# ryhorv/tf-flowavenet

Hardware: AMD Instinct MI355X
Metric: audio samples/sec: forward NLL + inverse synth, n_block=8 bf16 (higher is better)
Workload: dtype bf16; 1 GPU; configs[1]: full model n_block=8 n_flow=6 n_layer=2, forward NLL + inverse synthesis, 16128-sample (63-frame) clips @22.05 kHz; clips_per_gpu=8, samples_per_clip=16128, weights=synthetic seed 1234, ActNorm DDI on the first (global) batch, parallelism=batch shard x1, no data-path collective (2-scalar NLL all-reduce), streams=7 per direction

## Files before the change

### tf-flowavenet_amd/csrc/flow_kernels.hip

```cpp
#include "common.h"
#include "gemm_ring.h"
#include "fwn_internal.h"

struct RowCtxT {
    int row;
    int t;
};

struct FrontProb {
    static constexpr bool A_DMA = false;
    const float* xa;
    const float* an;
    const bf16* W;
    const float* bias;
    bf16* hout;
    int M, Ti, Ch, chlog, kpad, apply_an;
    unsigned char* h8out = nullptr;
    typedef RowCtxT RowCtx;
    struct ChunkCtx { int k0; int lo; };
    __device__ int nchunks() const { return 2 * (kpad / FWN_BK); }
    __device__ RowCtx row_ctx(int row) const { return RowCtx{row, row % Ti}; }
    __device__ ChunkCtx chunk_ctx(int q) const {
        const int nk = kpad / FWN_BK;
        const int lo = q >= nk;
// ... 540 lines not shown
                if (h8out) {
                    const srd_t s8 = make_srd(h8out, (uint32_t)((size_t)M * FWN_HID));
#pragma unroll
                    for (int r = 0; r < 16; r += 2) {
                        const unsigned int pk = pack_e4m3x2((float)(bf16)((hv[r] + acc[mi][ni][r] + b) * 0.70710678118654752f),
                                                            (float)(bf16)((hv[r + 1] + acc[mi][ni][r + 1] + b) * 0.70710678118654752f));
                        buf_store_u8(s8, voff >> 1, (uint32_t)((mi * 32 + acc_row_c(r)) * FWN_HID), pk);
                        buf_store_u8(s8, voff >> 1, (uint32_t)((mi * 32 + acc_row_c(r + 1)) * FWN_HID), pk >> 8);
                    }
                }
            }
        }
    }
};

struct CondProb {
    static constexpr bool NT_B = true;
    static constexpr bool A_DMA = true;
    static constexpr bool ALLOW_256 = false;
    const bf16* ca;
    const bf16* Wc;
    float* P;
    int M, cin, kcpad;
    int k_begin = 0, k_end = 0;
    struct RowCtx { int row; };
    struct ChunkCtx { int k0; };
    template <int BK> __device__ int nchunks() const { return ((k_end ? k_end : kcpad) - k_begin) / BK; }
    __device__ RowCtx row_ctx(int row) const { return RowCtx{row}; }
    template <int BK> __device__ ChunkCtx chunk_ctx(int q) const { return ChunkCtx{k_begin + q * BK}; }
    __device__ srd_t a_srd(const ChunkCtx&) const { return make_srd(ca, (uint32_t)((size_t)M * cin * 2)); }
    __device__ uint32_t a_voff(const ChunkCtx& cc, const RowCtx& rc, int c8) const {
        const bool ok = rc.row < M && cc.k0 + c8 * 8 < cin;
        return ok ? (uint32_t)(rc.row * cin + cc.k0 + c8 * 8) * 2u : FWN_OOB;
    }
    __device__ srd_t b_srd(const ChunkCtx&) const { return make_srd(Wc, (uint32_t)(512u * kcpad * 2u)); }
    __device__ uint32_t b_voff(const ChunkCtx& cc, int n, int c8) const {
        return (uint32_t)(n * kcpad + cc.k0 + c8 * 8) * 2u;
    }
    __device__ float acc_init(int) const { return 0.0f; }
    template <int MI>
    __device__ void epilogue(const f32x16 (&acc)[MI][2], int mrow0, int ncol0, int lane) const {
        const int lr = lane & 31;
        const srd_t sp = make_srd(P, (uint32_t)((size_t)M * 512 * 4));
#pragma unroll
        for (int ni = 0; ni < 2; ++ni) {
            const uint32_t voff = (uint32_t)((mrow0 + 4 * (lane >> 5)) * 512 + ncol0 + ni * 32 + lr) * 4u;
#pragma unroll
            for (int mi = 0; mi < MI; ++mi)
#pragma unroll
                for (int r = 0; r < 16; ++r)
                    buf_store_f32(sp, voff, (uint32_t)((mi * 32 + acc_row_c(r)) * 512 * 4), acc[mi][ni][r]);
        }
    }
};

template <int MI, class Prob>
__global__ __launch_bounds__(256) void gemm128_kernel(Prob p, int ntn) {
    const int wg = xcd_remap(blockIdx.x, gridDim.x);
    gemm128_body<MI, Prob>(p, wg / ntn, wg % ntn);
}

template <int BM, int BN, int WM, int WN, int BK, int D, class Prob, int KSP = 1>
__global__ __launch_bounds__(64 * WM * WN * KSP) void gemm_ring_kernel(Prob p, int ntn) {
    const int wg = xcd_remap(blockIdx.x, gridDim.x);
    gemm_ring_body<BM, BN, WM, WN, BK, D, Prob, KSP>(p, wg / ntn, wg % ntn);
}

struct CondBatch {
    const bf16* ca;
    const bf16* ca_odd;
    const bf16* Wc_base;
    float* P_base;
    long w_stride;
    long p_stride;
    int flow0, flow_step, L;
    int M, cin, kcpad;
    float* part_base;
    long part_stride;
    int nsplit;
};
template <int BM, int BN, int WM, int WN, int BK, int D>
__global__ __launch_bounds__(64 * WM * WN) void cond_batch_kernel(CondBatch cb, int ntn) {
    const int z = blockIdx.y;
    const int flow = cb.flow0 + (z / cb.L) * cb.flow_step;
    const int zi = flow * cb.L + (z % cb.L);
    const int sp = blockIdx.z;
    float* out = (sp == 0 ? cb.P_base : cb.part_base + (size_t)(sp - 1) * cb.part_stride) + (size_t)zi * cb.p_stride;
    CondProb p{(cb.ca_odd && (flow & 1)) ? cb.ca_odd : cb.ca, cb.Wc_base + (size_t)zi * cb.w_stride, out, cb.M, cb.cin, cb.kcpad};
    if (cb.nsplit > 1) {
        const int nch = cb.kcpad / 64, per = (nch + cb.nsplit - 1) / cb.nsplit;
        p.k_begin = min(sp * per, nch) * 64;
        p.k_end = min((sp + 1) * per, nch) * 64;
        if (p.k_end == 0) p.k_end = 64, p.k_begin = 64;
    }
    const int wg = xcd_remap(blockIdx.x, gridDim.x);
    gemm_ring_body<BM, BN, WM, WN, BK, D, CondProb>(p, wg / ntn, wg % ntn);
}


#include "tail_zero_prob.h"

struct TailLinProb {
    static constexpr bool A_DMA = true;
    static constexpr bool ALLOW_256 = false;
    const bf16* A;
    const bf16* W;
    const float* bias;
    bf16* out;
    long a_stride;
    int L, M;
    struct RowCtx { int row; };
    struct ChunkCtx { uint32_t abase; int bcol; };
    template <int BK> __device__ int nchunks() const { return L * FWN_HID / BK; }
    __device__ RowCtx row_ctx(int row) const { return RowCtx{row}; }
    template <int BK> __device__ ChunkCtx chunk_ctx(int q) const {
        constexpr int CPL = FWN_HID / BK;
        const int l = q / CPL, k0 = (q % CPL) * BK;
        return ChunkCtx{(uint32_t)(l * a_stride + k0), l * FWN_HID + k0};
    }
    __device__ srd_t a_srd(const ChunkCtx&) const { return make_srd(A, (uint32_t)(((size_t)(L - 1) * a_stride + (size_t)M * FWN_HID) * 2)); }
    __device__ uint32_t a_voff(const ChunkCtx& cc, const RowCtx& rc, int c8) const {
        return rc.row < M ? (cc.abase + (uint32_t)(rc.row * FWN_HID + c8 * 8)) * 2u : FWN_OOB;
    }
    __device__ srd_t b_srd(const ChunkCtx&) const { return make_srd(W, (uint32_t)(256u * L * FWN_HID * 2u)); }
    __device__ uint32_t b_voff(const ChunkCtx& cc, int n, int c8) const {
        return (uint32_t)(n * L * FWN_HID + cc.bcol + c8 * 8) * 2u;
    }
    __device__ float acc_init(int col) const { return bias[col]; }
    template <int MI>
    __device__ void epilogue(const f32x16 (&acc)[MI][2], int mrow0, int ncol0, int lane) const {
        const int lr = lane & 31;
        const srd_t so = make_srd(out, (uint32_t)((size_t)M * FWN_HID * 2));
#pragma unroll
        for (int ni = 0; ni < 2; ++ni) {
            const int col = swap_bits23(ncol0 + ni * 32 + lr);
            const uint32_t voff = (uint32_t)((mrow0 + 4 * (lane >> 5)) * FWN_HID + col) * 2u;
#pragma unroll
            for (int mi = 0; mi < MI; ++mi)
#pragma unroll
                for (int r = 0; r < 16; ++r)
                    buf_store_bf16(so, voff, (uint32_t)((mi * 32 + acc_row_c(r)) * FWN_HID * 2), fmaxf(acc[mi][ni][r], 0.0f));
        }
    }
};

#include "tail_chain.h"

constexpr int FWN_TAIL256_MIN = 192 * 256;
constexpr int FWN_TAIL_SPLIT_MAX = 12288;
constexpr int FWN_TAIL_SPLIT_CHAIN_MIN = 6144;
constexpr int FWN_TRS_MIN_ROWS = 1008;
constexpr int FWN_TRS_ROWS128 = 12288;
constexpr int FWN_TRS_ROWS64 = 6144;
constexpr int FWN_TRS_MAX_ROWS = 49152;
int fwn_tail_stream_min_rows() { return FWN_TRS_MIN_ROWS; }

constexpr int FWN_TAIL_ROWS256 = 256, FWN_TAIL_ROWS128 = 128, FWN_TAIL_ROWS_SPLIT = 64;
TailForm fwn_tail_form(int M, int L, int Ch, int npt, bool have_stream) {
    TailForm f{};
    if (have_stream && L == 2 && npt == 1 && Ch <= 32 && M >= FWN_TRS_MIN_ROWS && M < FWN_TRS_MAX_ROWS) {
        f.kind = TAIL_RS;
        f.rs_mt = M >= FWN_TRS_ROWS128 ? 4 : M >= FWN_TRS_ROWS64 ? 2 : 1;
        f.rows = 32 * f.rs_mt;
    } else if (M > FWN_TAIL_SPLIT_MAX) {
        f.kind = M >= FWN_TAIL256_MIN ? TAIL_FUSED256 : TAIL_FUSED128;
        f.rows = M >= FWN_TAIL256_MIN ? FWN_TAIL_ROWS256 : FWN_TAIL_ROWS128;
    } else {
        f.kind = M >= FWN_TAIL_SPLIT_CHAIN_MIN ? TAIL_SPLIT_CHAIN : TAIL_SPLIT3;
        f.rows = FWN_TAIL_ROWS_SPLIT;
        f.scratch = true;
    }
    f.xb_out = f.kind != TAIL_SPLIT3;
    f.front = f.xb_out && Ch <= 8 && npt == 1;
    return f;
}
int fwn_tail_slots(const TailForm& f, int M, bool front) {
    if (f.kind == TAIL_SPLIT3) return ((M + 63) / 64) * 8;
    const int rw = f.rows - (front ? 2 : 0);
    return (M + rw - 1) / rw;
}

int g_fwn_opt_rs_persist = -1;
int fwn_device_cus() {
    static int cache[64];
    int dev = 0;
    if (hipGetDevice(&dev) != hipSuccess || dev < 0 || dev >= 64) return 256;
    if (cache[dev] == 0) {
        int n = 0;
        if (hipDeviceGetAttribute(&n, hipDeviceAttributeMultiprocessorCount, dev) != hipSuccess || n < 2) n = 256;
        cache[dev] = n;
    }
    return cache[dev];
}

static inline int ilog2(int v) { int l = 0; while ((1 << l) < v) ++l; return l; }

template <class Prob>
static void launch_gemm128(const Prob& p, int M, int ntn, hipStream_t st) {
    const int t128 = (M + 127) / 128 * ntn;
    if (t128 >= 512) {
        hipLaunchKernelGGL((gemm128_kernel<2, Prob>), dim3(t128), dim3(256), 0, st, p, ntn);
    } else {
        const int t64 = (M + 63) / 64 * ntn;
        hipLaunchKernelGGL((gemm128_kernel<1, Prob>), dim3(t64), dim3(256), 0, st, p, ntn);
    }
}

#define RING_LAUNCH(BM, BN, WM, WN, BK, D) RING_LAUNCHK(BM, BN, WM, WN, BK, D, 1)
#define RING_LAUNCHK(BM, BN, WM, WN, BK, D, KSP)                                                    \
    hipLaunchKernelGGL((gemm_ring_kernel<BM, BN, WM, WN, BK, D, Prob, KSP>),                        \
                       dim3(((M + BM - 1) / BM) * (N / BN)), dim3(64 * WM * WN * KSP), 0, st, p, N / BN)
template <class Prob>
static void launch_ring(const Prob& p, int M, int N, int ksteps, hipStream_t st) {
    const int FILL = 192;
    if constexpr (Prob::ALLOW_256) {
        if (N % 256 == 0 && ((M + 255) / 256) * (N / 256) >= FILL) {
            RING_LAUNCH(256, 256, 4, 4, 64, 2);
            return;
        }
    }
    if (((M + 255) / 256) * (N / 128) >= FILL) {
        RING_LAUNCH(256, 128, 8, 2, 64, 3);
    } else if (((M + 127) / 128) * (N / 128) >= FILL) {
        RING_LAUNCH(128, 128, 4, 2, 64, 3);
    } else if (((M + 63) / 64) * (N / 128) >= FILL) {
        RING_LAUNCH(64, 128, 2, 2, 64, 4);
    } else {
        if (ksteps % 8 == 0) RING_LAUNCHK(64, 64, 2, 1, 128, 4, 4);
        else RING_LAUNCHK(64, 64, 2, 1, 64, 4, 2);
    }
}

void fwn_launch_front(const float* xa, const float* an_a, const void* W, const void* W2, const float* bias,
                      void* hout, void* scratch, int M, int Ti, int Ch, int kpad, int apply_an, void* h8out, hipStream_t st) {
    if (W2 && (Ch == 32 || Ch == 64 || Ch == 128 || (Ch == 16 && !h8out)) && ((uintptr_t)xa & 15) == 0) {
        const int grid = ((M + 63) / 64) * 4;
        if (Ch == 16) hipLaunchKernelGGL((front_mfma_kernel<32, 16>), dim3(grid), dim3(256), 0, st, xa, an_a, apply_an, (const bf16*)W2, bias, (bf16*)hout, M, Ti);
        else if (Ch == 32) hipLaunchKernelGGL((front_mfma_kernel<32>), dim3(grid), dim3(256), 0, st, xa, an_a, apply_an, (const bf16*)W2, bias, (bf16*)hout, M, Ti);
        else if (Ch == 64) hipLaunchKernelGGL((front_mfma_kernel<64>), dim3(grid), dim3(256), 0, st, xa, an_a, apply_an, (const bf16*)W2, bias, (bf16*)hout, M, Ti);
        else hipLaunchKernelGGL((front_mfma_kernel<128>), dim3(grid), dim3(256), 0, st, xa, an_a, apply_an, (const bf16*)W2, bias, (bf16*)hout, M, Ti);
        return;
    }
    if (Ch >= 32 && W2 && scratch) {
        const long total = (long)M * Ch;
        const int grid = (int)((total + 255) / 256 > 2048 ? 2048 : (total + 255) / 256);
        hipLaunchKernelGGL(xprep_kernel, dim3(grid), dim3(256), 0, st, xa, an_a, M, Ch, apply_an, (bf16*)scratch);
        FrontRingProb rp{(const bf16*)scratch, (const bf16*)W2, bias, (bf16*)hout, M, Ti, Ch};
        launch_ring(rp, M, 256, 6 * Ch / 16, st);
        return;
    }
    FrontProb p{xa, an_a, (const bf16*)W, bias, (bf16*)hout, M, Ti, Ch, ilog2(Ch), kpad, apply_an};
    if (Ch <= 16) {
        p.h8out = (unsigned char*)h8out;
#define FRONT_VALU(R, KMAX, ROWS) hipLaunchKernelGGL((front_valu_kernel<R, KMAX>), dim3((M + ROWS - 1) / ROWS), dim3(256), 0, st, p)
        const bool big = M >= 64 * 512;
        if (Ch <= 2) { if (big) FRONT_VALU(16, 6, 64); else FRONT_VALU(4, 6, 16); }
        else if (Ch <= 4) { if (big) FRONT_VALU(16, 12, 64); else FRONT_VALU(4, 12, 16); }
        else if (Ch <= 8) { if (big) FRONT_VALU(16, 24, 64); else FRONT_VALU(4, 24, 16); }
        else { if (big) FRONT_VALU(16, 48, 64); else FRONT_VALU(4, 48, 16); }
#undef FRONT_VALU
        return;
    }
    launch_gemm128(p, M, 2, st);
}

void fwn_launch_gate(const void* h, const void* ca, const float* P, const void* Wd, const void* Wc, const void* Wgs,
                     const float* bias, void* o, int M, int Ti, int dil, int cin, int kcpad, void* aux,
                     hipStream_t st) {
    if (Wgs && fwn_gate_stream_ok(M, Ti, dil, cin, ca != nullptr && P == nullptr, aux != nullptr)) {
        fwn_launch_gate_rs(h, ca, Wgs, bias, o, M, Ti, dil, cin, st);
        return;
    }
    GateProb p{(const bf16*)h, (const bf16*)ca, P, (const bf16*)Wd, (const bf16*)Wc, bias, (bf16*)o,
               M, Ti, dil, cin, kcpad};
    p.aux = (bf16*)aux;
    const int t256 = (M + 255) / 256;
    if (dil <= FWN_HALO_MAXDIL && t256 * 4 >= 192) {
        if (t256 * 2 >= 192)
            hipLaunchKernelGGL((gate_halo_kernel<256, 256, GateProb>), dim3(t256 * 2), dim3(1024), 0, st, p, 2);
        else
            hipLaunchKernelGGL((gate_halo_kernel<256, 128, GateProb>), dim3(t256 * 4), dim3(1024), 0, st, p, 4);
        return;
    }
    const int t128 = (M + 127) / 128;
    if (dil <= FWN_HALO_MAXDIL && t128 * 4 >= 192) {
        hipLaunchKernelGGL((gate_halo_kernel<128, 128, GateProb>), dim3(t128 * 4), dim3(512), 0, st, p, 4);
        return;
    }
    launch_ring(p, M, 512, (768 + (ca ? kcpad : 0)) / 16, st);
}

int fwn_gate_fp8_ok(int M, int dil) { return dil <= FWN_HALO_MAXDIL && ((M + 255) / 256) * 4 >= 192; }

void fwn_launch_gate_fp8(const void* h8, const void* ca, const void* Wd8, int wexp, const void* Wc, const float* bias, void* o,
                         int M, int Ti, int dil, int cin, int kcpad, hipStream_t st) {
    GateProb p{nullptr, (const bf16*)ca, nullptr, nullptr, (const bf16*)Wc, bias, (bf16*)o, M, Ti, dil, cin, kcpad};
    p.h8 = (const unsigned char*)h8;
    p.Wd8 = (const unsigned char*)Wd8;
    p.sb = 127 - wexp;
    const int t256 = (M + 255) / 256;
    if (t256 * 2 >= 192)
        hipLaunchKernelGGL((gate_halo_kernel<256, 256, GateProb, true>), dim3(t256 * 2), dim3(1024), 0, st, p, 2);
    else
        hipLaunchKernelGGL((gate_halo_kernel<256, 128, GateProb, true>), dim3(t256 * 4), dim3(1024), 0, st, p, 4);
}

void fwn_launch_res(const void* o, const void* hin, const void* W, const float* bias, void* hout, int M, void* h8out,
                    hipStream_t st) {
    ResProb p{(const bf16*)o, (const bf16*)hin, (const bf16*)W, bias, (bf16*)hout, M};
    p.h8out = (unsigned char*)h8out;
    if (((M + 255) / 256) * 2 >= 192) {
        const int N = 256;
        typedef ResProb Prob;
        RING_LAUNCH(128, 128, 4, 2, 64, 2);
        return;
// ... 131 lines not shown
```

### tf-flowavenet_amd/csrc/tail_rs.h

```cpp
#pragma once
#include "gate_rs.h"
#include "tail_chain.h"

#ifndef FWN_TRS_SAFE
#define FWN_TRS_SAFE 0
#endif
#ifndef FWN_TRS_ABL
#define FWN_TRS_ABL 0
#endif

#ifdef FWN_TRS_STAMP
#define TRS_STAMP(i) do { if (lane == 0) stamps[((size_t)blockIdx.x * 8 + wave) * 16 + (i)] = __builtin_amdgcn_s_memtime(); } while (0)
#define TRS_STAMP_RT(i) do { if (lane == 0) stamps[((size_t)blockIdx.x * 8 + wave) * 16 + (i)] = __builtin_amdgcn_s_memrealtime(); } while (0)
#define TRS_STAMP_ARG , unsigned long long* stamps
#else
#define TRS_STAMP(i) do { } while (0)
#define TRS_STAMP_RT(i) do { } while (0)
#define TRS_STAMP_ARG
#endif

__host__ __device__ constexpr int trs_default_r(int mt) { return mt >= 4 ? 8 : 12; }

template <int MT, int R, bool FRONT, bool SAVE>
struct TrsCount {
    static constexpr int PP = MT >= 2 ? MT / 2 : 1, WSLOT = MT > 1 ? 1 : 0;
    static constexpr int NKF = FRONT ? 3 : 0, NKW = 48 + NKF, NI = 8, LA = 3, NSV = SAVE ? 2 * MT : 0, NZ = 4, NX = 4;
    static_assert(R >= 3 && R - 1 <= 32, "ring depth");
    static constexpr int walk(int tk, int ta, int qk, int qa) {
        int count = -1, result = -1;
        bool done = false;
#define T_OP() do { if (count >= 0) ++count; } while (0)
#define T_W(k) do { T_OP(); if (tk == 0 && ta == (k)) count = 0; } while (0)
#define T_P1(i, j) do { T_OP(); if (tk == 1 && ta == (i) && (j) == PP - 1) count = 0; } while (0)
#define T_QK(g) do { if (!done && qk == 0 && qa == (g)) { result = count; done = true; } } while (0)
#define T_QB(i) do { if (!done && qk == 1 && qa == (i)) { result = count; done = true; } } while (0)
        T_OP();
        for (int k = 0; k < R - 1; ++k) {
            if (k % 2 == 0 && k / 2 < LA)
                for (int j = 0; j < PP; ++j) T_P1(k / 2, j);
            T_W(k);
        }
        for (int g = 0; g < 32; ++g) {
            T_QK(g);
            if ((g & 3) == 0) T_QB(g >> 2);
            for (int slot = 0; slot < MT; ++slot) {
                if ((g & 3) == 0 && slot < PP && (g >> 2) + LA < NI) T_P1((g >> 2) + LA, slot);
                if (slot == WSLOT && g + R - 1 < NKW) T_W(g + R - 1);
            }
        }
        for (int s = 0; s < NSV + NZ + NX; ++s) T_OP();
        for (int g = 32; g < 48; ++g) {
            T_QK(g);
            for (int slot = 0; slot < MT; ++slot)
                if (slot == WSLOT && g + R - 1 < NKW) T_W(g + R - 1);
        }
#undef T_OP
#undef T_W
#undef T_P1
#undef T_QK
#undef T_QB
        return result;
    }
    static constexpr int wait_kstep(int g) { return walk(0, g, 0, g); }
    static constexpr int wait_barrier(int i) { return walk(1, i, 1, i); }
};

typedef __attribute__((ext_vector_type(2))) __bf16 trs_bf16x2;
typedef __attribute__((ext_vector_type(2))) short trs_i16x2;
__device__ __forceinline__ uint32_t trs_relu_pk(f32x2 v) {
    const trs_i16x2 w = __builtin_bit_cast(trs_i16x2, __builtin_convertvector(v, trs_bf16x2));
    return __builtin_bit_cast(uint32_t, __builtin_elementwise_max(w, trs_i16x2{0, 0}));
}
__device__ __forceinline__ uint2 trs_pack4_relu(const f32x16& a, int q) {
    return make_uint2(trs_relu_pk(f32x2{a[4 * q], a[4 * q + 1]}), trs_relu_pk(f32x2{a[4 * q + 2], a[4 * q + 3]}));
}
__device__ __forceinline__ void trs_store_row32(const uint2 (&pk)[4], srd_t dst, uint32_t voff) {
#pragma unroll
    for (int p = 0; p < 2; ++p) {
        const auto s0 = __builtin_amdgcn_permlane32_swap(pk[2 * p].x, pk[2 * p + 1].x, false, false);
        const auto s1 = __builtin_amdgcn_permlane32_swap(pk[2 * p].y, pk[2 * p + 1].y, false, false);
        const u32x4 out = {s0[0], s1[0], s0[1], s1[1]};
        __builtin_amdgcn_raw_buffer_store_b128(out, dst, voff, p * 32, 0);
    }
}

__device__ __forceinline__ void trs_dma16(u32x4 srd, uint32_t voff, uint32_t lds_addr) {
    uint32_t keep;
    asm volatile("s_mov_b32 %0, m0\n\ts_mov_b32 m0, %3\n\ts_nop 4\n\tbuffer_load_dwordx4 %1, %2, 0 offen lds\n\ts_mov_b32 m0, %0"
                 : "=&s"(keep) : "v"(voff), "s"(srd), "s"(lds_addr) : "memory");
}
__device__ __forceinline__ u32x4 trs_srd(const void* p, uint32_t bytes) {
    const unsigned long long b = (unsigned long long)(uintptr_t)p;
    return u32x4{(uint32_t)__builtin_amdgcn_readfirstlane((int)(uint32_t)b), (uint32_t)__builtin_amdgcn_readfirstlane((int)(uint32_t)(b >> 32)) & 0xffffu,
                 (uint32_t)__builtin_amdgcn_readfirstlane((int)bytes), 0x00020000u};
}

__device__ __forceinline__ void trs_xload(float& dst, u32x4 srd, uint32_t voff) {
    asm volatile("s_nop 4\n\tbuffer_load_dword %0, %1, %2, 0 offen" : "=v"(dst) : "v"(voff), "s"(srd) : "memory");
}

template <int I, int R>
__device__ __forceinline__ void trs_touch(bf16x8 (&wq)[R]) {
    if constexpr (I < R) {
        asm volatile("" : "+v"(wq[I]));
        trs_touch<I + 1, R>(wq);
    }
}

template <int MT, bool FRONT, bool SAVE, int R = trs_default_r(MT)>
__global__ __launch_bounds__(512, (MT <= 2 ? 4 : 2)) void tail_rs_kernel(TailArgs a, const bf16* __restrict__ Wts TRS_STAMP_ARG) {
    using C = TrsCount<MT, R, FRONT, SAVE>;
    static_assert(MT == 1 || MT == 2 || MT == 4, "32-, 64- or 128-row tiles");
    static_assert(32 * MT * 512 >= 3 * MT * 1024, "the front conv's B fragments live in the U region");
    constexpr int BM = 32 * MT, PP = C::PP, WSLOT = C::WSLOT, NKW = C::NKW, NI = C::NI, LA = C::LA;
    constexpr int SLOT = BM * 128 > 8192 ? BM * 128 : 8192;
    constexpr int A_BYTES = 4 * SLOT > 32768 ? 4 * SLOT : 32768;
    constexpr int B_BYTES = BM * 512;
    constexpr int C_BS = 0, C_BF = 256, C_BZ = 512, C_EZ = 768, C_AN = 1024, C_BFN = 1280, C_ANN = 1536, CST = 2048;
    constexpr int T_FLOATS = FRONT ? BM * 8 : 0;
    __shared__ __attribute__((aligned(1024))) unsigned char lds[A_BYTES + B_BYTES + CST * 4 + T_FLOATS * 4 + 64];
    unsigned char* const lA = lds;
    const uint32_t lds0 = (uint32_t)__builtin_amdgcn_readfirstlane((int)(uint32_t)(uintptr_t)(lds_ptr_t)lds);
    unsigned char* const lB = lds + A_BYTES;
    float* const cst = (float*)(lds + A_BYTES + B_BYTES);
    float* const Tt = cst + CST;
    float* const red = Tt + T_FLOATS;

    const int tid = threadIdx.x, lane = tid & 63;
    const int wave = __builtin_amdgcn_readfirstlane(tid >> 6);
    const int lr = lane & 31, lh = lane >> 5;
    const int g0 = a.overlap ? (int)blockIdx.x * (BM - 2) - 1 : (int)blockIdx.x * BM;
    const int M = a.M, Ch = a.Ch;
    constexpr bool front = FRONT;
    TRS_STAMP(0); TRS_STAMP_RT(14);

    {
        const float* src = a.bs;
        uint32_t bytes = 0;
        if (wave == 0) { src = a.bs; bytes = 1024u; }
        else if (wave == 1) { src = a.bfin; bytes = 1024u; }
        else if (wave == 2) { src = a.bz; bytes = 256u; }
        else if (wave == 3) { src = a.ez; bytes = 256u; }
        else if (wave == 4) { src = a.an; bytes = (uint32_t)Ch * 32u; }
        else if (wave == 5 && front) { src = a.bfn; bytes = 1024u; }
        else if (wave == 6 && front && a.an_next) { src = a.an_next; bytes = (uint32_t)Ch * 32u; }
        trs_dma16(trs_srd(src, bytes), (uint32_t)lane * 16u, lds0 + (uint32_t)(A_BYTES + B_BYTES + 1024 * wave));
    }

    const u32x4 srd_o = trs_srd(a.o, (uint32_t)(((size_t)(a.L - 1) * a.o_stride + (size_t)M * FWN_HID) * 2));
    auto issue_piece = [&](int item, int j) {
        const int pi = wave + 8 * j;
        const int jrow = 8 * pi + (lane >> 3);
        const int c = (lane & 7) ^ ((jrow >> 1) & 7);
        const int gr = g0 + jrow;
        const bool ok = (jrow < BM) & ((unsigned)gr < (unsigned)M);
        const uint32_t off = (uint32_t)((item >> 2) * a.o_stride + (long)gr * FWN_HID + (item & 3) * 64 + c * 8) * 2u;
        trs_dma16(srd_o, ok ? off : FWN_OOB, lds0 + (uint32_t)((item & 3) * SLOT + (wave + 8 * j) * 1024));
    };

    const unsigned long long wbase = (unsigned long long)(uintptr_t)Wts + (unsigned long long)wave * (48 * 1024);
    const u32x4 wsrd = {(uint32_t)__builtin_amdgcn_readfirstlane((int)(uint32_t)wbase),
                        (uint32_t)__builtin_amdgcn_readfirstlane((int)(uint32_t)(wbase >> 32)) & 0xffffu, (uint32_t)(48 * 1024), 0x00020000u};
    const unsigned long long nbase = (unsigned long long)(uintptr_t)(front ? (const void*)a.Wfn : (const void*)Wts);
    const u32x4 nsrd = {(uint32_t)__builtin_amdgcn_readfirstlane((int)(uint32_t)nbase),
                        (uint32_t)__builtin_amdgcn_readfirstlane((int)(uint32_t)(nbase >> 32)) & 0xffffu,
                        front ? (uint32_t)(256 * a.kfn * 2) : 0u, 0x00020000u};
    const uint32_t wl = (uint32_t)lane * 16u;
    bf16x8 wq[R];
    auto issue_w = [&](auto G) {
        constexpr int g = decltype(G)::value;
        if constexpr (g < 48) {
            rs_wload<(g * 1024) % 4096>(wq[g % R], wsrd, (uint32_t)(((g * 1024) / 4096) * 4096), wl);
        } else {
            constexpr int kk = g - 48;
            const int col = kk * 16 + lh * 8;
            rs_wload<0>(wq[g % R], nsrd, 0u, col < a.kfn ? (uint32_t)(((wave * 32 + lr) * a.kfn + col) * 2) : FWN_OOB);
        }
    };
    auto wait_w = [&](auto G) {
        constexpr int g = decltype(G)::value;
        if (FWN_TRS_SAFE) rs_wwait<0>(wq[g % R]);
        else rs_wwait<C::wait_kstep(g)>(wq[g % R]);
    };

    rs_static_for<R - 1>([&](auto G) {
        constexpr int g = decltype(G)::value;
        if constexpr (g % 2 == 0 && g / 2 < LA) {
#pragma unroll
            for (int j = 0; j < PP; ++j) issue_piece(g / 2, j);
        }
        issue_w(G);
    });
    static_assert((R - 2) / 2 >= LA - 1, "the prologue issues the first LA slices among its weight loads");
    TRS_STAMP(1);

    f32x16 acc[MT];
    auto init_acc = [&](const float* bias, bool perm) {
#pragma unroll
        for (int q = 0; q < 4; ++q) {
            const int at = perm ? wave * 32 + 4 * (q & 1) + 8 * lh + 16 * (q >> 1) : wave * 32 + 8 * q + 4 * lh;
            const float4 v = *(const float4*)(bias + at);
#pragma unroll
            for (int mi = 0; mi < MT; ++mi) { acc[mi][4 * q] = v.x; acc[mi][4 * q + 1] = v.y; acc[mi][4 * q + 2] = v.z; acc[mi][4 * q + 3] = v.w; }
        }
    };
    bf16x8 hf[MT];
    const int rb1 = lr * 128, xv1 = (lh ^ ((lr >> 1) & 7)) << 4;
    const int rb2 = lr * 512, xv2 = (lh ^ (lr & 15)) << 4;
    auto kofs = [&](int x, int k32) {
        asm volatile("" : "+v"(x));
        return k32 ^ x;
    };
    auto su_off = [&](int mi, int q) { return lds_off256(mi * 32 + lr, wave * 4 + q) + 8 * lh; };
    const uint32_t su_bytes = (uint32_t)((size_t)M * FWN_HID * 2);
    auto row_of = [&](int mi) { return g0 + mi * 32 + lr; };
    auto owned_row = [&](int mi) {
        const int rl = mi * 32 + lr, row = g0 + rl;
        return (unsigned)row < (unsigned)M && (!a.overlap || (rl >= 1 && rl <= BM - 2));
    };
    auto park = [&](bf16* save) {
#pragma unroll
        for (int mi = 0; mi < MT; ++mi) {
            uint2 pk[4];
#pragma unroll
            for (int q = 0; q < 4; ++q) {
                pk[q] = trs_pack4_relu(acc[mi], q);
                *(uint2*)(lB + su_off(mi, q)) = pk[q];
            }
            if constexpr (SAVE)
                trs_store_row32(pk, make_srd(save, su_bytes), owned_row(mi) ? (uint32_t)(row_of(mi) * FWN_HID + wave * 32 + 8 * lh) * 2u : FWN_OOB);
        }
    };

    rs_static_for<32>([&](auto G) {
        constexpr int g = decltype(G)::value;
        constexpr int item = g >> 2, ki = g & 3;
        const unsigned char* la = lA + (item & 3) * SLOT;
        wait_w(G);
        if constexpr (ki == 0) {
            if (FWN_TRS_SAFE) rs_vmwait<0>(); else rs_vmwait<C::wait_barrier(item)>();
            FWN_RING_BARRIER();
            if constexpr (item == 0) { TRS_STAMP(2); init_acc(cst + C_BS, true); }
            const int ko = kofs(xv1, 0);
#pragma unroll
            for (int mi = 0; mi < MT; ++mi) hf[mi] = *(const bf16x8*)(la + rb1 + mi * 4096 + ko);
        }
        const int kon = ki < 3 ? kofs(xv1, (ki + 1) * 32) : 0;
        __builtin_amdgcn_sched_barrier(0);
        rs_static_for<MT>([&](auto MI) {
            constexpr int mi = decltype(MI)::value;
            acc[mi] = mfma32(wq[g % R], hf[mi], acc[mi]);
            if constexpr (ki < 3) hf[mi] = *(const bf16x8*)(la + rb1 + mi * 4096 + kon);
            if constexpr (ki == 0 && mi < PP && item + LA < NI) issue_piece(item + LA, mi);
            if constexpr (mi == WSLOT && g + R - 1 < NKW && FWN_TRS_ABL != 1) issue_w(std::integral_constant<int, g + R - 1>{});
            __builtin_amdgcn_sched_barrier(0);
        });
    });
    TRS_STAMP(3);
    park(a.save_s);
    FWN_RING_BARRIER();
    TRS_STAMP(4);
    {
        const u32x4 srd_z = trs_srd(a.Wz, 64u * 256u * 2u);
#pragma unroll
        for (int j = 0; j < 4; ++j) {
            const int pi = wave + 8 * j, q = pi >> 3;
            const int r = (pi & 7) * 8 + (lane >> 3);
            trs_dma16(srd_z, (uint32_t)(r * FWN_HID + q * 64 + ((lane & 7) ^ ((r >> 1) & 7)) * 8) * 2u, lds0 + (uint32_t)(pi * 1024));
        }
    }
    float xpre[4];
    {
        const unsigned long long xbase = (unsigned long long)(uintptr_t)a.xb;
        const u32x4 xsrd = {(uint32_t)__builtin_amdgcn_readfirstlane((int)(uint32_t)xbase),
                            (uint32_t)__builtin_amdgcn_readfirstlane((int)(uint32_t)(xbase >> 32)) & 0xffffu,
                            (uint32_t)((size_t)M * Ch * 4), 0x00020000u};
        const int row = g0 + wave * 32 + lr;
        const bool rv = (wave < MT) & ((unsigned)row < (unsigned)M);
#pragma unroll
        for (int r = 0; r < 4; ++r) {
            const int tau = r + 4 * lh;
            trs_xload(xpre[r], xsrd, (rv && tau < Ch) ? (uint32_t)(row * Ch + tau) * 4u : FWN_OOB);
        }
    }

    init_acc(cst + C_BF, true);
    rs_static_for<16>([&](auto G2) {
        constexpr int g2 = decltype(G2)::value, g = 32 + g2;
        wait_w(std::integral_constant<int, g>{});
        if constexpr (g2 == 0) {
            const int ko = kofs(xv2, 0);
#pragma unroll
            for (int mi = 0; mi < MT; ++mi) hf[mi] = *(const bf16x8*)(lB + rb2 + mi * 16384 + ko);
        }
        const int kon = g2 < 15 ? kofs(xv2, ((g2 + 1) & 7) * 32) + ((g2 + 1) >> 3) * 256 : 0;
        __builtin_amdgcn_sched_barrier(0);
        rs_static_for<MT>([&](auto MI) {
            constexpr int mi = decltype(MI)::value;
            acc[mi] = mfma32(wq[g % R], hf[mi], acc[mi]);
            if constexpr (g2 < 15) hf[mi] = *(const bf16x8*)(lB + rb2 + mi * 16384 + kon);
            if constexpr (mi == WSLOT && g + R - 1 < NKW && FWN_TRS_ABL != 1) issue_w(std::integral_constant<int, g + R - 1>{});
            __builtin_amdgcn_sched_barrier(0);
        });
    });
    TRS_STAMP(5);
    asm volatile("s_waitcnt vmcnt(0)" ::: "memory");
    __builtin_amdgcn_sched_barrier(0);
    trs_touch<0, R>(wq);
    asm volatile("" : "+v"(xpre[0]), "+v"(xpre[1]), "+v"(xpre[2]), "+v"(xpre[3]));
    TRS_STAMP(6);
    FWN_RING_BARRIER();
    TRS_STAMP(7);
    park(a.save_u);
    FWN_RING_BARRIER();
    TRS_STAMP(8);

    if (FWN_TRS_ABL == 2) return;
    const float* an_a = cst + C_AN;
    const float* an_b = an_a + 4 * Ch;
    const uint32_t plane_bytes = (uint32_t)((size_t)M * Ch * 4);
    float lsum = 0.0f;
    if (wave < MT) {
        f32x16 z0, z1;
#pragma unroll
        for (int r = 0; r < 16; ++r) { z0[r] = 0.0f; z1[r] = 0.0f; }
        const unsigned char* ub = lB + rb2 + wave * 16384;
        const unsigned char* zb = lA + lr * 128;
#pragma unroll
        for (int q = 0; q < 4; ++q)
#pragma unroll
            for (int kk = 0; kk < 4; ++kk) {
                const int g2 = 4 * q + kk;
                const bf16x8 b = *(const bf16x8*)(ub + (((g2 & 7) * 32) ^ xv2) + (g2 >> 3) * 256);
                const int wo = q * 8192 + (((kk * 2 + lh) ^ ((lr >> 1) & 7)) << 4);
                z0 = mfma32(*(const bf16x8*)(zb + wo), b, z0);
                z1 = mfma32(*(const bf16x8*)(zb + wo + 4096), b, z1);
            }
        TRS_STAMP(9);
        const int rl = wave * 32 + lr, row = g0 + rl;
        const bool rvalid = (unsigned)row < (unsigned)M;
        const bool owned = rvalid && (!a.overlap || (rl >= 1 && rl <= BM - 2));
        const float* bzl = cst + C_BZ;
        const float* ezl = cst + C_EZ;
        const float* ann = cst + C_ANN;
        const srd_t sxo = make_srd(a.xb_out ? a.xb_out : a.xb, plane_bytes);
        const bool vec4 = Ch >= 4;
        const srd_t sz = make_srd(a.save_z, SAVE && a.save_z ? (uint32_t)((size_t)M * 2 * Ch * 4) : 0u);
        float ov0[4];
        auto group = [&](auto Q, const float (&xq)[4]) {
            constexpr int q = decltype(Q)::value;
            const int j0 = 8 * q + 4 * lh;
            float bl[4], el[4], bt[4], et[4], s0[4], s1[4], s2[4], l3[4];
#pragma unroll
            for (int e = 0; e < 4; ++e) {
                const int j = j0 + e, tc = j < Ch ? j : 0;
                bl[e] = bzl[j]; el[e] = ezl[j]; bt[e] = bzl[j + 32]; et[e] = ezl[j + 32];
                s0[e] = an_b[tc];
                s1[e] = a.inverse ? an_b[2 * Ch + tc] : an_b[Ch + tc];
                l3[e] = a.inverse ? 0.0f : an_a[3 * Ch + tc] + an_b[3 * Ch + tc];
                s2[e] = 0.0f;
            }
            float ov[4];
#pragma unroll
            for (int e = 0; e < 4; ++e) {
                const int r = 4 * q + e, j = j0 + e;
                const bool ok = j < Ch && owned;
                const float ls = (z0[r] + bl[e]) * el[e];
                const float t = (z1[r] + bt[e]) * et[e];
                if (!a.inverse) {
                    const float yb = (xq[e] + s0[e]) * s1[e];
                    ov[e] = (yb - t) * __expf(-ls);
                    lsum += ok ? (l3[e] - ls) : 0.0f;
                } else {
                    const float yb = xq[e] * __expf(ls) + t;
                    ov[e] = yb * s1[e] - s0[e];
                }
            }
            if (vec4) {
                const uint32_t vo = (j0 < Ch && owned) ? (uint32_t)(row * Ch + j0) * 4u : FWN_OOB;
                const u32x4 o4 = {__builtin_bit_cast(unsigned int, ov[0]), __builtin_bit_cast(unsigned int, ov[1]),
                                  __builtin_bit_cast(unsigned int, ov[2]), __builtin_bit_cast(unsigned int, ov[3])};
                __builtin_amdgcn_raw_buffer_store_b128(o4, sxo, vo, 0, 0);
                if constexpr (SAVE) {
                    const uint32_t zoff = vo != FWN_OOB ? (uint32_t)(row * 2 * Ch + j0) * 4u : FWN_OOB;
                    u32x4 zl, zt;
#pragma unroll
                    for (int e = 0; e < 4; ++e) {
                        zl[e] = __builtin_bit_cast(unsigned int, z0[4 * q + e] + bl[e]);
                        zt[e] = __builtin_bit_cast(unsigned int, z1[4 * q + e] + bt[e]);
                    }
                    __builtin_amdgcn_raw_buffer_store_b128(zl, sz, zoff, 0, 0);
                    __builtin_amdgcn_raw_buffer_store_b128(zt, sz, zoff, Ch * 4, 0);
                }
            } else {
#pragma unroll
                for (int e = 0; e < 4; ++e) {
                    const int j = j0 + e;
                    const uint32_t vo = (j < Ch && owned) ? (uint32_t)(row * Ch + j) * 4u : FWN_OOB;
                    buf_store_f32(sxo, vo, 0, ov[e]);
                    if constexpr (SAVE) {
                        const uint32_t zoff = vo != FWN_OOB ? (uint32_t)(row * 2 * Ch + j) * 4u : FWN_OOB;
                        buf_store_f32(sz, zoff, 0, z0[4 * q + e] + bl[e]);
                        buf_store_f32(sz, zoff, Ch * 4, z1[4 * q + e] + bt[e]);
                    }
                }
            }
            if constexpr (q == 0) {
#pragma unroll
                for (int e = 0; e < 4; ++e) ov0[e] = ov[e];
            }
        };
        group(std::integral_constant<int, 0>{}, xpre);
        if (Ch > 8) {
            auto later = [&](auto Q) {
                constexpr int q = decltype(Q)::value;
                const int tau0 = 8 * q + 4 * lh;
                const float4 v = *(const float4*)(a.xb + ((tau0 < Ch && rvalid) ? (size_t)row * Ch + tau0 : 0));
                const float xq[4] = {v.x, v.y, v.z, v.w};
                group(Q, xq);
            };
            later(std::integral_constant<int, 1>{});
            if (Ch > 16) {
                later(std::integral_constant<int, 2>{});
                later(std::integral_constant<int, 3>{});
            }
        }
        if constexpr (FRONT) {
#pragma unroll
            for (int r = 0; r < 4; ++r) {
                const int tau = r + 4 * lh;
                if (tau < Ch) {
                    const float v = a.an_next ? (ov0[r] + ann[tau]) * ann[Ch + tau] : ov0[r];
                    Tt[rl * 8 + tau] = rvalid ? v : 0.0f;
                }
            }
        }
        if (a.partial) {
#pragma unroll
            for (int s = 32; s > 0; s >>= 1) lsum += __shfl_xor(lsum, s);
            if (lane == 0) red[wave] = lsum;
        }
    } else {
        constexpr int NT = 512 - 64 * MT;
        const int t2 = tid - 64 * MT;
        const srd_t sxa = make_srd(a.xa, plane_bytes);
        const int ra = max(a.overlap ? g0 + 1 : g0, 0), rb = min(a.overlap ? g0 + BM - 1 : g0 + BM, M);
        const int total = (rb - ra) * Ch;
        const uint32_t base = (uint32_t)(ra * Ch) * 4u;
        const int chmask = Ch - 1;
        if (Ch >= 4) {
            for (int idx = t2 * 4; idx < total; idx += NT * 4) {
                const float4 v = *(const float4*)(a.xa + (size_t)ra * Ch + idx);
                float f[4] = {v.x, v.y, v.z, v.w};
#pragma unroll
                for (int e = 0; e < 4; ++e) {
                    const int tau = (idx + e) & chmask;
                    f[e] = a.inverse ? (f[e] * an_a[2 * Ch + tau] - an_a[tau]) : ((f[e] + an_a[tau]) * an_a[Ch + tau]);
                }
                const u32x4 o4 = {__builtin_bit_cast(unsigned int, f[0]), __builtin_bit_cast(unsigned int, f[1]),
                                  __builtin_bit_cast(unsigned int, f[2]), __builtin_bit_cast(unsigned int, f[3])};
                __builtin_amdgcn_raw_buffer_store_b128(o4, sxa, base + (uint32_t)idx * 4u, 0, 0);
            }
        } else {
            for (int idx = t2; idx < total; idx += NT) {
                const int tau = idx & chmask;
                const uint32_t off = base + (uint32_t)idx * 4u;
                const float v = buf_load_f32(sxa, off, 0);
                buf_store_f32(sxa, off, 0, a.inverse ? (v * an_a[2 * Ch + tau] - an_a[tau]) : ((v + an_a[tau]) * an_a[Ch + tau]));
            }
        }
    }
    TRS_STAMP(10);
    if (a.partial == nullptr && !FRONT) { TRS_STAMP_RT(15); return; }
    asm volatile("s_waitcnt lgkmcnt(0)" ::: "memory");
    __builtin_amdgcn_s_barrier();
    asm volatile("" ::: "memory");
    TRS_STAMP(11);
    if (a.partial && tid == 0) {
        float t = 0.0f;
        for (int w = 0; w < MT; ++w) t += red[w];
        a.partial[blockIdx.x] = t;
    }
    if constexpr (FRONT) {
        init_acc(cst + C_BFN, false);
        const int chlog = 31 - __builtin_clz(Ch);
        const int nks = a.kfn >> 4;
        for (int f = wave; f < MT * nks; f += 8) {
            const int mi = f & (MT - 1), kk = f / MT;
            const int rl = mi * 32 + lr, row = g0 + rl;
            const bool rvalid = (unsigned)row < (unsigned)M;
            const int t_in = rvalid ? row % a.Ti : 0;
            Pack16 b;
#pragma unroll
            for (int e = 0; e < 4; ++e) {
                const int idx = kk * 8 + lh * 4 + e;
                const int tap = idx >> chlog, tau = idx & (Ch - 1);
                const int rr = rl + tap - 1;
                const bool ok = idx < 3 * Ch && (unsigned)(t_in + tap - 1) < (unsigned)a.Ti && (unsigned)rr < (unsigned)BM;
                const float v = ok ? Tt[(ok ? rr : 0) * 8 + tau] : 0.0f;
                const bf16 hi = (bf16)v;
                b.e[2 * e] = hi;
                b.e[2 * e + 1] = (bf16)(v - (float)hi);
            }
            *(uint4*)(lB + f * 1024 + lane * 16) = b.u;
        }
        asm volatile("s_waitcnt lgkmcnt(0)" ::: "memory");
        __builtin_amdgcn_s_barrier();
        asm volatile("" ::: "memory");
        rs_static_for<3>([&](auto KK) {
            constexpr int kk = decltype(KK)::value;
            if (kk < nks) {
#pragma unroll
                for (int mi = 0; mi < MT; ++mi)
                    acc[mi] = mfma32(wq[(48 + kk) % R], *(const bf16x8*)(lB + (kk * MT + mi) * 1024 + lane * 16), acc[mi]);
            }
        });
        TRS_STAMP(12);
        const srd_t sh = make_srd(a.h0_next, su_bytes);
#pragma unroll
        for (int mi = 0; mi < MT; ++mi) {
            uint2 pk[4];
#pragma unroll
            for (int q = 0; q < 4; ++q) pk[q] = trs_pack4_relu(acc[mi], q);
            trs_store_row32(pk, sh, owned_row(mi) ? (uint32_t)(row_of(mi) * FWN_HID + wave * 32 + 8 * lh) * 2u : FWN_OOB);
        }
    }
    TRS_STAMP(13); TRS_STAMP_RT(15);
}

struct TailStreamJob { const bf16* Ws; const bf16* Wf; bf16* out; };
__global__ void tail_stream_pack_kernel(const bf16* __restrict__ Ws, const bf16* __restrict__ Wf, bf16* __restrict__ out,
                                        const TailStreamJob* __restrict__ jobs) {
    if (jobs) {
        const TailStreamJob j = jobs[blockIdx.y];
        Ws = j.Ws; Wf = j.Wf; out = j.out;
    }
    const long total = 8L * 48 * 64;
    for (long i = blockIdx.x * (long)blockDim.x + threadIdx.x; i < total; i += (long)gridDim.x * blockDim.x) {
        const int lane = (int)(i & 63);
        const long t = i >> 6;
        const int g = (int)(t % 48), w = (int)(t / 48);
        const int ch = w * 32 + (lane & 31);
        const int prow = (ch & ~12) | ((ch & 4) << 1) | ((ch & 8) >> 1);
        const int col = (g < 32 ? g : g - 32) * 16 + 8 * (lane >> 5);
        ((uint4*)out)[i] = g < 32 ? *(const uint4*)(Ws + (size_t)prow * 512 + col) : *(const uint4*)(Wf + (size_t)prow * 256 + col);
    }
}
```

### tf-flowavenet_amd/csrc/tail_rs.hip

```cpp
#include "tail_rs.h"
#include "fwn_internal.h"

long fwn_tail_stream_size(int L) { return L == 2 ? 8L * 48 * 1024 : 0; }

void fwn_launch_tail_stream_pack(const void* Ws, const void* Wf, void* out, hipStream_t st) {
    hipLaunchKernelGGL(tail_stream_pack_kernel, dim3(96), dim3(256), 0, st, (const bf16*)Ws, (const bf16*)Wf, (bf16*)out, (const TailStreamJob*)nullptr);
}
void fwn_launch_tail_stream_pack_jobs(const void* jobs, int njobs, hipStream_t st) {
    hipLaunchKernelGGL(tail_stream_pack_kernel, dim3(24, njobs), dim3(256), 0, st, (const bf16*)nullptr, (const bf16*)nullptr, (bf16*)nullptr,
                       (const TailStreamJob*)jobs);
}

void fwn_launch_tail_rs(const TailArgs& a, const void* Wts, int mt, hipStream_t st) {
    const bool front = a.h0_next != nullptr, save = a.save_s && a.save_u && a.save_z;
    const int rows = 32 * mt - (a.overlap ? 2 : 0);
    const dim3 grid((a.M + rows - 1) / rows), block(512);
#define TRS_LAUNCH(MT)                                                                                                       \
    do {                                                                                                                     \
        if (front) hipLaunchKernelGGL((tail_rs_kernel<MT, true, false>), grid, block, 0, st, a, (const bf16*)Wts);           \
        else if (save) hipLaunchKernelGGL((tail_rs_kernel<MT, false, true>), grid, block, 0, st, a, (const bf16*)Wts);       \
        else hipLaunchKernelGGL((tail_rs_kernel<MT, false, false>), grid, block, 0, st, a, (const bf16*)Wts);                \
    } while (0)
    if (mt == 4) TRS_LAUNCH(4);
    else if (mt == 2) TRS_LAUNCH(2);
    else TRS_LAUNCH(1);
#undef TRS_LAUNCH
}
```

Measured before the change: 49.64 million samples/s.

## Add 256-row tail_rs tile with aliased LDS for large small-channel layers

Adds an MT=8 (256-row) variant of the streaming tail kernel and routes layers with M >= 49152 and Ch <= 8 to it instead of the fused tail path. To fit LDS, the o ring and the S/U image share one region, Wz gets its own small slice, S parking is split around a barrier, and all waves do both the z GEMM and the xa pass. The ring depth drops to 6. This aims to reuse weights across more rows per block, at the cost of fewer resident workgroups and extra barriers.

```diff
diff --git a/tf-flowavenet_amd/csrc/flow_kernels.hip b/tf-flowavenet_amd/csrc/flow_kernels.hip
--- a/tf-flowavenet_amd/csrc/flow_kernels.hip
+++ b/tf-flowavenet_amd/csrc/flow_kernels.hip
@@ -716,15 +716,16 @@
 constexpr int FWN_TRS_MIN_ROWS = 1008;
 constexpr int FWN_TRS_ROWS128 = 12288;
 constexpr int FWN_TRS_ROWS64 = 6144;
-constexpr int FWN_TRS_MAX_ROWS = 49152;
+constexpr int FWN_TRS_ROWS256 = 49152;
+constexpr int FWN_TRS_ROWS256_MAX_CH = 8;
 int fwn_tail_stream_min_rows() { return FWN_TRS_MIN_ROWS; }
 
 constexpr int FWN_TAIL_ROWS256 = 256, FWN_TAIL_ROWS128 = 128, FWN_TAIL_ROWS_SPLIT = 64;
 TailForm fwn_tail_form(int M, int L, int Ch, int npt, bool have_stream) {
     TailForm f{};
-    if (have_stream && L == 2 && npt == 1 && Ch <= 32 && M >= FWN_TRS_MIN_ROWS && M < FWN_TRS_MAX_ROWS) {
+    if (have_stream && L == 2 && npt == 1 && Ch <= 32 && M >= FWN_TRS_MIN_ROWS && (M < FWN_TRS_ROWS256 || Ch <= FWN_TRS_ROWS256_MAX_CH)) {
         f.kind = TAIL_RS;
-        f.rs_mt = M >= FWN_TRS_ROWS128 ? 4 : M >= FWN_TRS_ROWS64 ? 2 : 1;
+        f.rs_mt = M >= FWN_TRS_ROWS256 ? 8 : M >= FWN_TRS_ROWS128 ? 4 : M >= FWN_TRS_ROWS64 ? 2 : 1;
         f.rows = 32 * f.rs_mt;
     } else if (M > FWN_TAIL_SPLIT_MAX) {
         f.kind = M >= FWN_TAIL256_MIN ? TAIL_FUSED256 : TAIL_FUSED128;
diff --git a/tf-flowavenet_amd/csrc/tail_rs.h b/tf-flowavenet_amd/csrc/tail_rs.h
--- a/tf-flowavenet_amd/csrc/tail_rs.h
+++ b/tf-flowavenet_amd/csrc/tail_rs.h
@@ -19,13 +19,14 @@
 #define TRS_STAMP_ARG
 #endif
 
-__host__ __device__ constexpr int trs_default_r(int mt) { return mt >= 4 ? 8 : 12; }
+__host__ __device__ constexpr int trs_default_r(int mt) { return mt >= 8 ? 6 : mt >= 4 ? 8 : 12; }
 
 template <int MT, int R, bool FRONT, bool SAVE>
 struct TrsCount {
     static constexpr int PP = MT >= 2 ? MT / 2 : 1, WSLOT = MT > 1 ? 1 : 0;
-    static constexpr int NKF = FRONT ? 3 : 0, NKW = 48 + NKF, NI = 8, LA = 3, NSV = SAVE ? 2 * MT : 0, NZ = 4, NX = 4;
+    static constexpr int NKF = FRONT ? 3 : 0, NKW = 48 + NKF, NI = 8, LA = 3, NSV = SAVE ? 2 * MT : 0, NZ = MT == 8 ? 1 : 4, NX = 4;
     static_assert(R >= 3 && R - 1 <= 32, "ring depth");
+    static_assert(MT == 1 || (PP <= MT && PP * 8 * 8 == 32 * MT), "a wave's PP pieces of 8 rows cover an o slice and ride the MFMA slots of one k-step");
     static constexpr int walk(int tk, int ta, int qk, int qa) {
         int count = -1, result = -1;
         bool done = false;
@@ -110,19 +111,26 @@
 template <int MT, bool FRONT, bool SAVE, int R = trs_default_r(MT)>
 __global__ __launch_bounds__(512, (MT <= 2 ? 4 : 2)) void tail_rs_kernel(TailArgs a, const bf16* __restrict__ Wts TRS_STAMP_ARG) {
     using C = TrsCount<MT, R, FRONT, SAVE>;
-    static_assert(MT == 1 || MT == 2 || MT == 4, "32-, 64- or 128-row tiles");
+    static_assert(MT == 1 || MT == 2 || MT == 4 || MT == 8, "32-, 64-, 128- or 256-row tiles");
     static_assert(32 * MT * 512 >= 3 * MT * 1024, "the front conv's B fragments live in the U region");
     constexpr int BM = 32 * MT, PP = C::PP, WSLOT = C::WSLOT, NKW = C::NKW, NI = C::NI, LA = C::LA;
     constexpr int SLOT = BM * 128 > 8192 ? BM * 128 : 8192;
     constexpr int A_BYTES = 4 * SLOT > 32768 ? 4 * SLOT : 32768;
     constexpr int B_BYTES = BM * 512;
+    constexpr bool UNION = MT == 8;
+    constexpr int B_OFF = UNION ? 0 : A_BYTES, Z_OFF = UNION ? A_BYTES : 0, Z_BYTES = UNION ? 8192 : 0;
+    constexpr int C_OFF = UNION ? A_BYTES + Z_BYTES : A_BYTES + B_BYTES;
+    static_assert(!UNION || A_BYTES == B_BYTES, "one region for the o ring and the S / U image");
     constexpr int C_BS = 0, C_BF = 256, C_BZ = 512, C_EZ = 768, C_AN = 1024, C_BFN = 1280, C_ANN = 1536, CST = 2048;
     constexpr int T_FLOATS = FRONT ? BM * 8 : 0;
-    __shared__ __attribute__((aligned(1024))) unsigned char lds[A_BYTES + B_BYTES + CST * 4 + T_FLOATS * 4 + 64];
+    constexpr int LDS_BYTES = C_OFF + CST * 4 + T_FLOATS * 4 + 64;
+    static_assert(LDS_BYTES <= 160 * 1024, "LDS of one workgroup (MT = 8, FRONT: 128 + 8 + 8 + 8 KB + 64 = 155 712 bytes)");
+    __shared__ __attribute__((aligned(1024))) unsigned char lds[LDS_BYTES];
     unsigned char* const lA = lds;
     const uint32_t lds0 = (uint32_t)__builtin_amdgcn_readfirstlane((int)(uint32_t)(uintptr_t)(lds_ptr_t)lds);
-    unsigned char* const lB = lds + A_BYTES;
-    float* const cst = (float*)(lds + A_BYTES + B_BYTES);
+    unsigned char* const lB = lds + B_OFF;
+    unsigned char* const lZ = lds + Z_OFF;
+    float* const cst = (float*)(lds + C_OFF);
     float* const Tt = cst + CST;
     float* const red = Tt + T_FLOATS;
 
@@ -144,7 +152,7 @@
         else if (wave == 4) { src = a.an; bytes = (uint32_t)Ch * 32u; }
         else if (wave == 5 && front) { src = a.bfn; bytes = 1024u; }
         else if (wave == 6 && front && a.an_next) { src = a.an_next; bytes = (uint32_t)Ch * 32u; }
-        trs_dma16(trs_srd(src, bytes), (uint32_t)lane * 16u, lds0 + (uint32_t)(A_BYTES + B_BYTES + 1024 * wave));
+        trs_dma16(trs_srd(src, bytes), (uint32_t)lane * 16u, lds0 + (uint32_t)(C_OFF + 1024 * wave));
     }
 
     const u32x4 srd_o = trs_srd(a.o, (uint32_t)(((size_t)(a.L - 1) * a.o_stride + (size_t)M * FWN_HID) * 2));
@@ -218,9 +226,9 @@
         const int rl = mi * 32 + lr, row = g0 + rl;
         return (unsigned)row < (unsigned)M && (!a.overlap || (rl >= 1 && rl <= BM - 2));
     };
-    auto park = [&](bf16* save) {
-#pragma unroll
-        for (int mi = 0; mi < MT; ++mi) {
+    auto park = [&](bf16* save, int m_lo, int m_hi) {
+#pragma unroll
+        for (int mi = m_lo; mi < m_hi; ++mi) {
             uint2 pk[4];
 #pragma unroll
             for (int q = 0; q < 4; ++q) {
@@ -257,10 +265,20 @@
         });
     });
     TRS_STAMP(3);
-    park(a.save_s);
+    if constexpr (UNION) {
+        park(a.save_s, 0, 6);
+        FWN_RING_BARRIER();
+        park(a.save_s, 6, 8);
+    } else {
+        park(a.save_s, 0, MT);
+    }
     FWN_RING_BARRIER();
     TRS_STAMP(4);
-    {
+    if constexpr (UNION) {
+        const u32x4 srd_z = trs_srd(a.Wz, 64u * 256u * 2u);
+        const int q = wave >> 1, r8 = lane >> 3, r = (wave & 1) * 32 + r8;
+        trs_dma16(srd_z, (uint32_t)(r * FWN_HID + q * 64 + ((lane & 7) ^ ((r8 >> 1) & 7)) * 8) * 2u, lds0 + (uint32_t)(Z_OFF + wave * 1024));
+    } else {
         const u32x4 srd_z = trs_srd(a.Wz, 64u * 256u * 2u);
 #pragma unroll
         for (int j = 0; j < 4; ++j) {
@@ -311,7 +329,7 @@
     TRS_STAMP(6);
     FWN_RING_BARRIER();
     TRS_STAMP(7);
-    park(a.save_u);
+    park(a.save_u, 0, MT);
     FWN_RING_BARRIER();
     TRS_STAMP(8);
 
@@ -320,21 +338,23 @@
     const float* an_b = an_a + 4 * Ch;
     const uint32_t plane_bytes = (uint32_t)((size_t)M * Ch * 4);
     float lsum = 0.0f;
-    if (wave < MT) {
+    const bool tile_wave = UNION || wave < MT;
+    if (tile_wave) {
         f32x16 z0, z1;
 #pragma unroll
         for (int r = 0; r < 16; ++r) { z0[r] = 0.0f; z1[r] = 0.0f; }
         const unsigned char* ub = lB + rb2 + wave * 16384;
-        const unsigned char* zb = lA + lr * 128;
+        const int zr = UNION ? (lr & 7) : lr;
+        const unsigned char* zb = lZ + zr * 128;
 #pragma unroll
         for (int q = 0; q < 4; ++q)
 #pragma unroll
             for (int kk = 0; kk < 4; ++kk) {
                 const int g2 = 4 * q + kk;
                 const bf16x8 b = *(const bf16x8*)(ub + (((g2 & 7) * 32) ^ xv2) + (g2 >> 3) * 256);
-                const int wo = q * 8192 + (((kk * 2 + lh) ^ ((lr >> 1) & 7)) << 4);
+                const int wo = q * (UNION ? 2048 : 8192) + (((kk * 2 + lh) ^ ((zr >> 1) & 7)) << 4);
                 z0 = mfma32(*(const bf16x8*)(zb + wo), b, z0);
-                z1 = mfma32(*(const bf16x8*)(zb + wo + 4096), b, z1);
+                z1 = mfma32(*(const bf16x8*)(zb + wo + (UNION ? 1024 : 4096)), b, z1);
             }
         TRS_STAMP(9);
         const int rl = wave * 32 + lr, row = g0 + rl;
@@ -440,9 +460,10 @@
             for (int s = 32; s > 0; s >>= 1) lsum += __shfl_xor(lsum, s);
             if (lane == 0) red[wave] = lsum;
         }
-    } else {
-        constexpr int NT = 512 - 64 * MT;
-        const int t2 = tid - 64 * MT;
+    }
+    if (UNION || !tile_wave) {
+        constexpr int NT = UNION ? 512 : 512 - 64 * MT;
+        const int t2 = UNION ? tid : tid - 64 * MT;
         const srd_t sxa = make_srd(a.xa, plane_bytes);
         const int ra = max(a.overlap ? g0 + 1 : g0, 0), rb = min(a.overlap ? g0 + BM - 1 : g0 + BM, M);
         const int total = (rb - ra) * Ch;
diff --git a/tf-flowavenet_amd/csrc/tail_rs.hip b/tf-flowavenet_amd/csrc/tail_rs.hip
--- a/tf-flowavenet_amd/csrc/tail_rs.hip
+++ b/tf-flowavenet_amd/csrc/tail_rs.hip
@@ -21,7 +21,8 @@
         else if (save) hipLaunchKernelGGL((tail_rs_kernel<MT, false, true>), grid, block, 0, st, a, (const bf16*)Wts);       \
         else hipLaunchKernelGGL((tail_rs_kernel<MT, false, false>), grid, block, 0, st, a, (const bf16*)Wts);                \
     } while (0)
-    if (mt == 4) TRS_LAUNCH(4);
+    if (mt == 8) TRS_LAUNCH(8);
+    else if (mt == 4) TRS_LAUNCH(4);
     else if (mt == 2) TRS_LAUNCH(2);
     else TRS_LAUNCH(1);
 #undef TRS_LAUNCH
```

Result: no change. 50.07 million samples/s, median of 6 (+0.9%).
